# Hongje/OTVM

Hardware: AMD Instinct MI355X
Metric: frames_per_sec (higher is better)
Workload: dtype f16x3 (fp32 operands split into fp16 hi+lo, fp32 accumulate); 1 GPU; synthetic 1920x1080 clip, T=140 frames (untimed lead-in 0 + warmup 5 + timed: the last 135), memory every 5, max 5 slots, trimap propagation + alpha + memorize per frame, one sequence per GPU; weights=synthetic (otvm_amd.synth_weights seed 0), parallelism=sequence-per-gpu x1, batch=1

## Files before the change

### otvm_amd/csrc/gram.hip

```cpp
#include "common.h"
#include "f16x3_ops.h"
#include <stdlib.h>

namespace {

struct GramArgs {
    const float* x; int64_t P; int C, ld;
    const float* in_scale; const float* in_shift; float in_slope;
    float* gpart; float* spart;
    int nk, pch, nblk, nb;
    int64_t x_bs, g_bs, s_bs; int norm_bs;
    unsigned* diag;
};

constexpr int LDT = 40;

template <int BS, int PASSES>
__global__ __launch_bounds__(BS == 256 ? 512 : 256, BS == 256 ? 1 : 2) void gram_f16_kernel(const GramArgs pa) {
    GramArgs p = pa;
    {
        const int zb = blockIdx.y;
        p.x += zb * p.x_bs;
        p.gpart += zb * p.g_bs;
        p.spart += zb * p.s_bs;
        if (p.in_scale) { p.in_scale += zb * p.norm_bs; p.in_shift += zb * p.norm_bs; }
    }
    const int xcd = blockIdx.x & 7, slot = blockIdx.x >> 3;
    const int kc = xcd + 8 * (slot / p.nblk), blk = slot % p.nblk;
    if (kc >= p.nk) return;
    constexpr int NT = BS == 256 ? 512 : 256;
    constexpr int WM = BS == 256 ? 4 : 2, WN = 2;
    constexpr int TM = BS / (32 * WM), TN = BS / (32 * WN);
    constexpr int ROWS = 2 * BS;
    constexpr int STAGE = ROWS * LDT * (PASSES == 3 ? 2 : 1);
    __shared__ __attribute__((aligned(16))) _Float16 smem[2 * STAGE];
    const int tid = threadIdx.x, lane = tid & 63, wave = tid >> 6, wm = wave / WN, wn = wave % WN;
    int bi = 0, bj = 0;
    {
        int b = blk;
        while (b >= p.nb - bi) { b -= p.nb - bi; ++bi; }
        bj = bi + b;
    }
    const bool diag = bi == bj;
    const int boff = diag ? 0 : BS;
    const int64_t p0 = (int64_t)kc * p.pch;
    const int64_t p1 = p0 + p.pch < p.P ? p0 + p.pch : p.P;
    const int nchunks = (int)((p1 - p0 + 31) >> 5);

    constexpr int MAXIT = ((2 * BS / 4) * 8 + NT - 1) / NT;
    const int NQ = (diag ? BS : 2 * BS) / 4;
    const int pg = tid & 7;
    int row0[MAXIT], chan[MAXIT];
    bool live[MAXIT];
    f32x4 sc[MAXIT], sh[MAXIT], ssum[MAXIT];
#pragma unroll
    for (int k = 0; k < MAXIT; ++k) {
        const int cq = (tid >> 3) + (NT / 8) * k;
        live[k] = cq < NQ;
        row0[k] = cq * 4;
        chan[k] = live[k] ? (cq * 4 < BS ? bi * BS + cq * 4 : bj * BS + cq * 4 - BS) : 0;
        sc[k] = f32x4{1.f, 1.f, 1.f, 1.f};
        sh[k] = f32x4{0.f, 0.f, 0.f, 0.f};
        if (p.in_scale && live[k]) {
            sc[k] = *reinterpret_cast<const f32x4*>(p.in_scale + chan[k]);
            sh[k] = *reinterpret_cast<const f32x4*>(p.in_shift + chan[k]);
        }
        ssum[k] = f32x4{0.f, 0.f, 0.f, 0.f};
    }
    constexpr int PF = 2;
    f32x4 rg[PF][MAXIT][4];
    auto load_chunk = [&](int c, f32x4 (&r)[MAXIT][4]) __attribute__((always_inline)) {
#pragma unroll
        for (int k = 0; k < MAXIT; ++k)
#pragma unroll
            for (int i = 0; i < 4; ++i) {
                int64_t px = p0 + (int64_t)c * 32 + pg * 4 + i;
                px = px < p1 ? px : p1 - 1;
                r[k][i] = *reinterpret_cast<const f32x4*>(p.x + px * p.ld + chan[k]);
            }
    };
    bool sat = false;
    auto store_chunk = [&](int c, int buf, f32x4 (&r)[MAXIT][4]) __attribute__((always_inline)) {
        _Float16* Th = smem + buf * STAGE;
        _Float16* Tl = Th + ROWS * LDT;
#pragma unroll
        for (int k = 0; k < MAXIT; ++k) {
            if (!live[k]) continue;
            f32x4 v[4];
#pragma unroll
            for (int i = 0; i < 4; ++i) {
                const bool ok = p0 + (int64_t)c * 32 + pg * 4 + i < p1;
                f32x4 t = r[k][i] * sc[k] + sh[k];
                t.x = t.x > 0.f ? t.x : t.x * p.in_slope; t.y = t.y > 0.f ? t.y : t.y * p.in_slope;
                t.z = t.z > 0.f ? t.z : t.z * p.in_slope; t.w = t.w > 0.f ? t.w : t.w * p.in_slope;
                const f32x4 z = {0.f, 0.f, 0.f, 0.f};
                t = ok ? t : z;
                const f32x4 c4 = {__builtin_amdgcn_fmed3f(t.x, -65504.f, 65504.f), __builtin_amdgcn_fmed3f(t.y, -65504.f, 65504.f),
                                  __builtin_amdgcn_fmed3f(t.z, -65504.f, 65504.f), __builtin_amdgcn_fmed3f(t.w, -65504.f, 65504.f)};
                sat |= (c4.x != t.x) | (c4.y != t.y) | (c4.z != t.z) | (c4.w != t.w);
                v[i] = c4;
                ssum[k] += v[i];
            }
#pragma unroll
            for (int j = 0; j < 4; ++j) {
                const f16x4 hi = {(_Float16)v[0][j], (_Float16)v[1][j], (_Float16)v[2][j], (_Float16)v[3][j]};
                *reinterpret_cast<f16x4*>(&Th[(row0[k] + j) * LDT + pg * 4]) = hi;
                if (PASSES == 3) {
                    const f16x4 lo = {(_Float16)(v[0][j] - (float)hi.x), (_Float16)(v[1][j] - (float)hi.y),
                                      (_Float16)(v[2][j] - (float)hi.z), (_Float16)(v[3][j] - (float)hi.w)};
                    *reinterpret_cast<f16x4*>(&Tl[(row0[k] + j) * LDT + pg * 4]) = lo;
                }
            }
        }
    };
    f32x16 acc[TM][TN];
#pragma unroll
    for (int a = 0; a < TM; ++a)
#pragma unroll
        for (int b = 0; b < TN; ++b)
#pragma unroll
            for (int e = 0; e < 16; ++e) acc[a][b][e] = 0.f;
    auto compute = [&](int buf) __attribute__((always_inline)) {
        const _Float16* Th = smem + buf * STAGE;
        const _Float16* Tl = Th + ROWS * LDT;
        const int frow = lane & 31, fk = (lane >> 5) * 8;
#pragma unroll
        for (int ks = 0; ks < 2; ++ks) {
            f16x8 ah[TM], bh[TN], al[TM], bl[TN];
#pragma unroll
            for (int a = 0; a < TM; ++a) {
                const int o = ((wm * TM + a) * 32 + frow) * LDT + 16 * ks + fk;
                ah[a] = *reinterpret_cast<const f16x8*>(&Th[o]);
                if (PASSES == 3) al[a] = *reinterpret_cast<const f16x8*>(&Tl[o]);
            }
#pragma unroll
            for (int b = 0; b < TN; ++b) {
                const int o = (boff + (wn * TN + b) * 32 + frow) * LDT + 16 * ks + fk;
                bh[b] = *reinterpret_cast<const f16x8*>(&Th[o]);
                if (PASSES == 3) bl[b] = *reinterpret_cast<const f16x8*>(&Tl[o]);
            }
            if (PASSES == 3) {
#pragma unroll
                for (int a = 0; a < TM; ++a)
#pragma unroll
                    for (int b = 0; b < TN; ++b) acc[a][b] = __builtin_amdgcn_mfma_f32_32x32x16_f16(al[a], bh[b], acc[a][b], 0, 0, 0);
#pragma unroll
                for (int a = 0; a < TM; ++a)
#pragma unroll
                    for (int b = 0; b < TN; ++b) acc[a][b] = __builtin_amdgcn_mfma_f32_32x32x16_f16(ah[a], bl[b], acc[a][b], 0, 0, 0);
            }
#pragma unroll
            for (int a = 0; a < TM; ++a)
#pragma unroll
                for (int b = 0; b < TN; ++b) acc[a][b] = __builtin_amdgcn_mfma_f32_32x32x16_f16(ah[a], bh[b], acc[a][b], 0, 0, 0);
        }
    };

    if (nchunks > 0) {
        load_chunk(0, rg[0]);
        load_chunk(1, rg[1]);
        store_chunk(0, 0, rg[0]);
        load_chunk(2, rg[0]);
        __syncthreads();
        for (int c = 0; c < nchunks; c += PF) {
#pragma unroll
            for (int j = 0; j < PF; ++j) {
                if (c + j >= nchunks) break;
                compute((c + j) & 1);
                if (c + j + 1 < nchunks) store_chunk(c + j + 1, (c + j + 1) & 1, rg[(j + 1) % PF]);
                load_chunk(c + j + 3, rg[(j + 1) % PF]);
                __syncthreads();
            }
        }
    }
    if (sat && p.diag) atomicOr(p.diag + 1, 2u);
    float* gp = p.gpart + ((int64_t)kc * p.nblk + blk) * (BS * BS);
    const int col = lane & 31, rbase = (lane >> 5) * 4;
#pragma unroll
    for (int a = 0; a < TM; ++a)
#pragma unroll
        for (int b = 0; b < TN; ++b)
#pragma unroll
            for (int e = 0; e < 16; ++e) {
                const int m = (wm * TM + a) * 32 + (e & 3) + 8 * (e >> 2) + rbase, n = (wn * TN + b) * 32 + col;
                gp[m * BS + n] = acc[a][b][e];
            }
    if (diag) {
#pragma unroll
        for (int k = 0; k < MAXIT; ++k) {
            f32x4 s = ssum[k];
#pragma unroll
            for (int off = 1; off < 8; off <<= 1) {
                s.x += __shfl_xor(s.x, off); s.y += __shfl_xor(s.y, off); s.z += __shfl_xor(s.z, off); s.w += __shfl_xor(s.w, off);
            }
            if (live[k] && pg == 0) *reinterpret_cast<f32x4*>(p.spart + (int64_t)kc * p.C + chan[k]) = s;
        }
    }
}

struct PredArgs {
    const float* gpart; const float* spart; int nk, E, C;
    const float* Mp; const double* v;
    double* ws; unsigned* counter;
    int64_t P; int Cout;
    const float* wscale; const float* gamma; const float* beta; const float* res_shift;
    float* scale_eff; float* bias_eff; float* stat_out;
    int64_t g_bs, s_bs; int ws_bs, tab_bs, rs_bs;
    unsigned* diag;
};

constexpr int PRED_WG = 1024;
constexpr int PRED_KP = 4;
__global__ __launch_bounds__(256) void gn_predict_kernel(const PredArgs pa) {
    PredArgs p = pa;
    const int zb = blockIdx.y;
    p.gpart += zb * p.g_bs;
    p.spart += zb * p.s_bs;
    p.ws += (int64_t)zb * p.ws_bs;
    const int tid = threadIdx.x, lane = tid & 63, kp = tid >> 6;
    __shared__ double part[PRED_KP][64][4];
    __shared__ double red[4][64];
    __shared__ float t_mean[32], t_rstd[32];
    __shared__ unsigned t_last;
    const int nq = p.E >> 2;
    double a2[8] = {0.0, 0.0, 0.0, 0.0, 0.0, 0.0, 0.0, 0.0};
    for (int q0 = blockIdx.x * 64; q0 < nq; q0 += gridDim.x * 64) {
        const int q = q0 + lane;
        const float* gp = p.gpart + 4 * (int64_t)q;
        double s4[4] = {0.0, 0.0, 0.0, 0.0};
        for (int k0 = kp; k0 < p.nk; k0 += 8 * PRED_KP) {
            f32x4 u[8];
#pragma unroll
            for (int j = 0; j < 8; ++j) {
                const int kk = k0 + j * PRED_KP;
                u[j] = *reinterpret_cast<const f32x4*>(gp + (int64_t)(kk < p.nk ? kk : p.nk - 1) * p.E);
            }
#pragma unroll
            for (int j = 0; j < 8; ++j) {
                if (k0 + j * PRED_KP < p.nk) {
                    s4[0] += (double)u[j].x; s4[1] += (double)u[j].y; s4[2] += (double)u[j].z; s4[3] += (double)u[j].w;
                }
            }
        }
        __syncthreads();
#pragma unroll
        for (int j = 0; j < 4; ++j) part[kp][lane][j] = s4[j];
        __syncthreads();
        double g4[4];
#pragma unroll
        for (int j = 0; j < 4; ++j) g4[j] = (part[0][lane][j] + part[1][lane][j]) + (part[2][lane][j] + part[3][lane][j]);
        f32x4 m[8];
#pragma unroll
        for (int j = 0; j < 8; ++j) m[j] = *reinterpret_cast<const f32x4*>(p.Mp + (int64_t)(kp * 8 + j) * p.E + 4 * (int64_t)q);
#pragma unroll
        for (int j = 0; j < 8; ++j)
            a2[j] += (g4[0] * (double)m[j].x + g4[1] * (double)m[j].y) + (g4[2] * (double)m[j].z + g4[3] * (double)m[j].w);
    }
    double a1[8] = {0.0, 0.0, 0.0, 0.0, 0.0, 0.0, 0.0, 0.0};
    if ((int)blockIdx.x * 64 < p.C) {
        const int c = blockIdx.x * 64 + lane;
        double sv = 0.0;
        if (c < p.C)
            for (int k = kp; k < p.nk; k += PRED_KP) sv += (double)p.spart[(int64_t)k * p.C + c];
        __syncthreads();
        part[kp][lane][0] = sv;
        __syncthreads();
        const double st = (part[0][lane][0] + part[1][lane][0]) + (part[2][lane][0] + part[3][lane][0]);
        if (c < p.C) {
#pragma unroll
            for (int j = 0; j < 8; ++j) a1[j] = st * p.v[(int64_t)(kp * 8 + j) * p.C + c];
        }
    }
#pragma unroll
    for (int j = 0; j < 8; ++j) {
        double x = a2[j], y = a1[j];
#pragma unroll
        for (int off = 32; off > 0; off >>= 1) {
            x += __shfl_xor(x, off);
            y += __shfl_xor(y, off);
        }
        if (lane == 0) { red[0][2 * (kp * 8 + j)] = y; red[0][2 * (kp * 8 + j) + 1] = x; }
    }
    __syncthreads();
    if (tid < 64) __hip_atomic_store(p.ws + (int64_t)blockIdx.x * 64 + tid, red[0][tid], __ATOMIC_RELAXED, __HIP_MEMORY_SCOPE_AGENT);
    __builtin_amdgcn_fence(__ATOMIC_RELEASE, "workgroup");
    __builtin_amdgcn_s_waitcnt(0);
    __syncthreads();
    if (tid == 0) t_last = atomicAdd(p.counter + zb, 1u) == gridDim.x - 1 ? 1u : 0u;
    __syncthreads();
    if (!t_last) return;
    {
        const int vi = tid & 63, ph = tid >> 6, n = (int)gridDim.x;
        double t = 0.0;
        for (int w0 = ph; w0 < n; w0 += 32) {
            double u[8];
#pragma unroll
            for (int j = 0; j < 8; ++j) {
                const int w = w0 + 4 * j;
                u[j] = __hip_atomic_load(p.ws + (int64_t)(w < n ? w : n - 1) * 64 + vi, __ATOMIC_RELAXED, __HIP_MEMORY_SCOPE_AGENT);
            }
#pragma unroll
            for (int j = 0; j < 8; ++j)
                if (w0 + 4 * j < n) t += u[j];
        }
        red[ph][vi] = t;
    }
    __syncthreads();
    const int cg = p.Cout / 32;
    if (tid < 32) {
        const double cnt = (double)p.P * cg;
        const double sum = (red[0][2 * tid] + red[1][2 * tid]) + (red[2][2 * tid] + red[3][2 * tid]);
        const double sq = (red[0][2 * tid + 1] + red[1][2 * tid + 1]) + (red[2][2 * tid + 1] + red[3][2 * tid + 1]);
        const double mean = sum / cnt;
        double var = sq / cnt - mean * mean;
        if (var < 0.0) var = 0.0;
        t_mean[tid] = (float)mean;
        t_rstd[tid] = (float)(1.0 / sqrt(var + 1e-5));
        if (p.diag) {
            const double kappa = mean * mean / (var + 1e-12);
            const bool bad = !(sum == sum) || !(sq == sq) || !(fabs(sum) < 1e300) || !(fabs(sq) < 1e300);
            if (bad) atomicOr(p.diag + 1, 1u);
            else atomicMax(p.diag, __float_as_uint((float)(kappa < 3e38 ? kappa : 3e38)));
        }
        if (p.stat_out) { p.stat_out[zb * 64 + 2 * tid] = t_mean[tid]; p.stat_out[zb * 64 + 2 * tid + 1] = t_rstd[tid]; }
    }
    __syncthreads();
    float* se = p.scale_eff + (int64_t)zb * p.tab_bs;
    float* be = p.bias_eff + (int64_t)zb * p.tab_bs;
    const float* rs = p.res_shift ? p.res_shift + (int64_t)zb * p.rs_bs : nullptr;
    for (int c = tid; c < p.Cout; c += 256) {
        const int g = c / cg;
        const float a = t_rstd[g] * p.gamma[c];
        se[c] = p.wscale[c] * a;
        float b = p.beta[c] - t_mean[g] * a;
        if (rs) b += rs[c];
        be[c] = b;
    }
    if (tid == 0) __hip_atomic_store(p.counter + zb, 0u, __ATOMIC_RELAXED, __HIP_MEMORY_SCOPE_AGENT);
}

}

extern "C" int otvm_gram_block(int C) {
    static const int cap = otvm_probe_int("OTVM_GRAM_BS", 128);
    if (C % 256 == 0 && cap >= 256) return 256;
    return C % 128 == 0 && cap >= 128 ? 128 : 64;
}

extern "C" int64_t otvm_gram_entries(int C) {
    const int bs = otvm_gram_block(C), nb = C / bs;
    return (int64_t)(nb * (nb + 1) / 2) * bs * bs;
}

extern "C" int otvm_gram_chunks(int64_t P, int C, int* pch_out) {
    const int bs = otvm_gram_block(C), nb = C / bs, nblk = nb * (nb + 1) / 2;
    static const int wgs = otvm_probe_int("OTVM_GRAM_WGS", 0);
    int64_t nk = (wgs > 0 ? wgs : (bs == 256 ? 192 : 384)) / nblk;
    if (nk > 128) nk = 128;
    if (nk > P / 256) nk = P / 256;
    if (nk < (P + 1023) / 1024) nk = (P + 1023) / 1024;
    if (nk < 1) nk = 1;
    int64_t pch = (P + nk - 1) / nk;
    pch = (pch + 31) / 32 * 32;
    nk = (P + pch - 1) / pch;
    if (pch_out) *pch_out = (int)pch;
    return (int)nk;
}

extern "C" int64_t otvm_gn_predict_ws_bytes(void) { return (int64_t)PRED_WG * 64 * sizeof(double); }

extern "C" int otvm_gram_f16(const otvm_gram_params* q, void* stream) {
    OTVM_REQUIRE(q && q->x && q->gpart && q->spart, "otvm_gram_f16: null pointer");
    OTVM_REQUIRE(q->C % 64 == 0 && q->C >= 64 && q->ld % 4 == 0 && q->ld >= q->C && ((uintptr_t)q->x & 15) == 0,
                 "otvm_gram_f16: C must be a multiple of 64 in a 16-byte aligned view (C %d, ld %d)", q->C, q->ld);
    OTVM_REQUIRE(!q->in_scale == !q->in_shift, "otvm_gram_f16: in_scale and in_shift go together");
    OTVM_REQUIRE(q->passes == 1 || q->passes == 3, "otvm_gram_f16: passes must be 1 (fp16) or 3 (f16x3)");
    GramArgs a;
    a.x = q->x; a.P = q->P; a.C = q->C; a.ld = q->ld;
    a.in_scale = q->in_scale; a.in_shift = q->in_shift;
    a.in_slope = q->in_act == OTVM_ACT_RELU ? 0.f : (q->in_act == OTVM_ACT_LEAKY ? 0.01f : 1.f);
    a.gpart = q->gpart; a.spart = q->spart;
    const int bs = otvm_gram_block(q->C);
    a.nb = q->C / bs; a.nblk = a.nb * (a.nb + 1) / 2;
    int pch = 0;
    a.nk = otvm_gram_chunks(q->P, q->C, &pch);
    a.pch = pch;
    const int batch = q->batch > 1 ? q->batch : 1;
    a.x_bs = batch > 1 ? q->x_bs : 0; a.norm_bs = batch > 1 ? q->norm_bs : 0;
    a.g_bs = (int64_t)a.nk * otvm_gram_entries(q->C); a.s_bs = (int64_t)a.nk * q->C;
    a.diag = q->diag;
    const dim3 grid(a.nblk * ((a.nk + 7) / 8) * 8, batch);
    hipStream_t s = (hipStream_t)stream;
    const bool p3 = q->passes == 3;
    if (bs == 256) {
        if (p3) hipLaunchKernelGGL((gram_f16_kernel<256, 3>), grid, dim3(512), 0, s, a);
        else hipLaunchKernelGGL((gram_f16_kernel<256, 1>), grid, dim3(512), 0, s, a);
    } else if (bs == 128) {
        if (p3) hipLaunchKernelGGL((gram_f16_kernel<128, 3>), grid, dim3(256), 0, s, a);
        else hipLaunchKernelGGL((gram_f16_kernel<128, 1>), grid, dim3(256), 0, s, a);
    } else {
        if (p3) hipLaunchKernelGGL((gram_f16_kernel<64, 3>), grid, dim3(256), 0, s, a);
        else hipLaunchKernelGGL((gram_f16_kernel<64, 1>), grid, dim3(256), 0, s, a);
    }
    OTVM_CHECK_LAUNCH("otvm_gram_f16");
    return 0;
}

extern "C" int otvm_gn_predict(const otvm_gn_predict_params* q, void* stream) {
    OTVM_REQUIRE(q && q->gpart && q->spart && q->Mp && q->v && q->ws && q->counter && q->wscale && q->gamma && q->beta &&
                     q->scale_eff && q->bias_eff, "otvm_gn_predict: null pointer");
    OTVM_REQUIRE(q->Cout % 32 == 0 && q->C % 64 == 0, "otvm_gn_predict: Cout must be a multiple of 32 (got %d)", q->Cout);
    OTVM_REQUIRE(((uintptr_t)q->Mp & 15) == 0 && ((uintptr_t)q->gpart & 15) == 0, "otvm_gn_predict: Mp / gpart must be 16-byte aligned");
    PredArgs a;
    a.gpart = q->gpart; a.spart = q->spart; a.C = q->C;
    a.E = (int)otvm_gram_entries(q->C);
    a.nk = otvm_gram_chunks(q->P, q->C, nullptr);
    a.Mp = q->Mp; a.v = q->v; a.ws = (double*)q->ws; a.counter = q->counter;
    a.P = q->P; a.Cout = q->Cout;
    a.wscale = q->wscale; a.gamma = q->gamma; a.beta = q->beta; a.res_shift = q->res_shift;
    a.scale_eff = q->scale_eff; a.bias_eff = q->bias_eff; a.stat_out = q->stat_out;
    const int batch = q->batch > 1 ? q->batch : 1;
    a.g_bs = (int64_t)a.nk * a.E; a.s_bs = (int64_t)a.nk * q->C;
    a.ws_bs = PRED_WG * 64; a.tab_bs = batch > 1 ? q->tab_bs : 0; a.rs_bs = batch > 1 ? q->rs_bs : 0;
    a.diag = q->diag;
    int nwg = a.E / 256;
    if (nwg > 192) nwg = 192;
    if (nwg < otvm_ceil_div(a.C, 64)) nwg = otvm_ceil_div(a.C, 64);
    hipLaunchKernelGGL(gn_predict_kernel, dim3(nwg, batch), dim3(256), 0, (hipStream_t)stream, a);
    OTVM_CHECK_LAUNCH("otvm_gn_predict");
    return 0;
}
```

Measured before the change: 48.55 frames/s.

## Split GN-predict reduction over K chunks and retune gram prefetch and chunking

The gn_predict kernel now splits its reduction over gram chunks across more workgroups, spreading the per-channel sum work over several split groups and prefetching Mp, spart and v early. The final reduction gets wider phases, and affine parameters are preloaded before the last-block wait. The gram kernel gets a configurable prefetch depth per block size, 3 waves per SIMD for BS=128, and a halved block when BS equals C. The chunk-count heuristic now targets resident occupancy. Together these aim to raise parallelism and cut latency in the GroupNorm statistic prediction, at the cost of register pressure and more partial sums.

Result: no change. 48.86 frames/s, median of 6 (+0.6%).

```diff
diff --git a/otvm_amd/csrc/gram.hip b/otvm_amd/csrc/gram.hip
--- a/otvm_amd/csrc/gram.hip
+++ b/otvm_amd/csrc/gram.hip
@@ -13,10 +13,20 @@
     unsigned* diag;
 };
 
+#ifndef OTVM_GRAM_PF64
+#define OTVM_GRAM_PF64 2
+#endif
+#ifndef OTVM_GRAM_PF128
+#define OTVM_GRAM_PF128 1
+#endif
+#ifndef OTVM_GRAM_WG128
+#define OTVM_GRAM_WG128 3
+#endif
+constexpr int GRAM_PF(int bs) { return bs == 64 ? OTVM_GRAM_PF64 : (bs == 128 ? OTVM_GRAM_PF128 : 2); }
 constexpr int LDT = 40;
 
 template <int BS, int PASSES>
-__global__ __launch_bounds__(BS == 256 ? 512 : 256, BS == 256 ? 1 : 2) void gram_f16_kernel(const GramArgs pa) {
+__global__ __launch_bounds__(BS == 256 ? 512 : 256, BS == 256 ? 1 : (BS == 128 ? OTVM_GRAM_WG128 : 2)) void gram_f16_kernel(const GramArgs pa) {
     GramArgs p = pa;
     {
         const int zb = blockIdx.y;
@@ -67,7 +77,7 @@
         }
         ssum[k] = f32x4{0.f, 0.f, 0.f, 0.f};
     }
-    constexpr int PF = 2;
+    constexpr int PF = GRAM_PF(BS);
     f32x4 rg[PF][MAXIT][4];
     auto load_chunk = [&](int c, f32x4 (&r)[MAXIT][4]) __attribute__((always_inline)) {
 #pragma unroll
@@ -157,10 +167,10 @@
     };
 
     if (nchunks > 0) {
-        load_chunk(0, rg[0]);
-        load_chunk(1, rg[1]);
+#pragma unroll
+        for (int j = 0; j < PF; ++j) load_chunk(j, rg[j]);
         store_chunk(0, 0, rg[0]);
-        load_chunk(2, rg[0]);
+        load_chunk(PF, rg[0]);
         __syncthreads();
         for (int c = 0; c < nchunks; c += PF) {
 #pragma unroll
@@ -168,7 +178,7 @@
                 if (c + j >= nchunks) break;
                 compute((c + j) & 1);
                 if (c + j + 1 < nchunks) store_chunk(c + j + 1, (c + j + 1) & 1, rg[(j + 1) % PF]);
-                load_chunk(c + j + 3, rg[(j + 1) % PF]);
+                load_chunk(c + j + 1 + PF, rg[(j + 1) % PF]);
                 __syncthreads();
             }
         }
@@ -200,6 +210,8 @@
 
 struct PredArgs {
     const float* gpart; const float* spart; int nk, E, C;
+    int nqb, ksplit, kper;
+    int kss, kper_s;
     const float* Mp; const double* v;
     double* ws; unsigned* counter;
     int64_t P; int Cout;
@@ -210,7 +222,13 @@
 };
 
 constexpr int PRED_WG = 1024;
+constexpr int PRED_ITEMS = 768;
+constexpr int PRED_SPLIT_WG = 128;
+constexpr int PRED_KMIN = 32;
 constexpr int PRED_KP = 4;
+constexpr int PRED_TP = 8;
+constexpr int PRED_TB = 16;
+constexpr int PRED_TQ = 8;
 __global__ __launch_bounds__(256) void gn_predict_kernel(const PredArgs pa) {
     PredArgs p = pa;
     const int zb = blockIdx.y;
@@ -219,25 +237,49 @@
     p.ws += (int64_t)zb * p.ws_bs;
     const int tid = threadIdx.x, lane = tid & 63, kp = tid >> 6;
     __shared__ double part[PRED_KP][64][4];
-    __shared__ double red[4][64];
+    __shared__ double red[PRED_TP][64];
     __shared__ float t_mean[32], t_rstd[32];
     __shared__ unsigned t_last;
-    const int nq = p.E >> 2;
+    const int ncb = p.C >> 6;
+    const bool has_s = (int)blockIdx.x < ncb * p.kss;
+    const float* sp = p.spart;
+    int s_lo = 0, s_hi = 1;
+    float us[8] = {0.f, 0.f, 0.f, 0.f, 0.f, 0.f, 0.f, 0.f};
+    double vv[8] = {0.0, 0.0, 0.0, 0.0, 0.0, 0.0, 0.0, 0.0};
+    if (has_s) {
+        const int c = ((int)blockIdx.x % ncb) * 64 + lane;
+        const int k_lo = ((int)blockIdx.x / ncb) * p.kper_s;
+        s_lo = k_lo + kp;
+        s_hi = k_lo + p.kper_s < p.nk ? k_lo + p.kper_s : p.nk;
+        sp += c;
+#pragma unroll
+        for (int j = 0; j < 8; ++j) {
+            const int kk = s_lo + j * PRED_KP;
+            us[j] = sp[(int64_t)(kk < s_hi ? kk : s_hi - 1) * p.C];
+        }
+#pragma unroll
+        for (int j = 0; j < 8; ++j) vv[j] = p.v[(int64_t)(kp * 8 + j) * p.C + c];
+    }
     double a2[8] = {0.0, 0.0, 0.0, 0.0, 0.0, 0.0, 0.0, 0.0};
-    for (int q0 = blockIdx.x * 64; q0 < nq; q0 += gridDim.x * 64) {
-        const int q = q0 + lane;
+    const int items = p.nqb * p.ksplit;
+    for (int it = blockIdx.x; it < items; it += gridDim.x) {
+        const int q = (it % p.nqb) * 64 + lane;
+        const int k_lo = (it / p.nqb) * p.kper, k_hi = k_lo + p.kper < p.nk ? k_lo + p.kper : p.nk;
+        f32x4 m[8];
+#pragma unroll
+        for (int j = 0; j < 8; ++j) m[j] = *reinterpret_cast<const f32x4*>(p.Mp + (int64_t)(kp * 8 + j) * p.E + 4 * (int64_t)q);
         const float* gp = p.gpart + 4 * (int64_t)q;
         double s4[4] = {0.0, 0.0, 0.0, 0.0};
-        for (int k0 = kp; k0 < p.nk; k0 += 8 * PRED_KP) {
+        for (int k0 = k_lo + kp; k0 < k_hi; k0 += 8 * PRED_KP) {
             f32x4 u[8];
 #pragma unroll
             for (int j = 0; j < 8; ++j) {
                 const int kk = k0 + j * PRED_KP;
-                u[j] = *reinterpret_cast<const f32x4*>(gp + (int64_t)(kk < p.nk ? kk : p.nk - 1) * p.E);
+                u[j] = *reinterpret_cast<const f32x4*>(gp + (int64_t)(kk < k_hi ? kk : k_hi - 1) * p.E);
             }
 #pragma unroll
             for (int j = 0; j < 8; ++j) {
-                if (k0 + j * PRED_KP < p.nk) {
+                if (k0 + j * PRED_KP < k_hi) {
                     s4[0] += (double)u[j].x; s4[1] += (double)u[j].y; s4[2] += (double)u[j].z; s4[3] += (double)u[j].w;
                 }
             }
@@ -249,27 +291,33 @@
         double g4[4];
 #pragma unroll
         for (int j = 0; j < 4; ++j) g4[j] = (part[0][lane][j] + part[1][lane][j]) + (part[2][lane][j] + part[3][lane][j]);
-        f32x4 m[8];
-#pragma unroll
-        for (int j = 0; j < 8; ++j) m[j] = *reinterpret_cast<const f32x4*>(p.Mp + (int64_t)(kp * 8 + j) * p.E + 4 * (int64_t)q);
 #pragma unroll
         for (int j = 0; j < 8; ++j)
             a2[j] += (g4[0] * (double)m[j].x + g4[1] * (double)m[j].y) + (g4[2] * (double)m[j].z + g4[3] * (double)m[j].w);
     }
     double a1[8] = {0.0, 0.0, 0.0, 0.0, 0.0, 0.0, 0.0, 0.0};
-    if ((int)blockIdx.x * 64 < p.C) {
-        const int c = blockIdx.x * 64 + lane;
+    if (has_s) {
         double sv = 0.0;
-        if (c < p.C)
-            for (int k = kp; k < p.nk; k += PRED_KP) sv += (double)p.spart[(int64_t)k * p.C + c];
+#pragma unroll
+        for (int j = 0; j < 8; ++j)
+            if (s_lo + j * PRED_KP < s_hi) sv += (double)us[j];
+        for (int k0 = s_lo + 8 * PRED_KP; k0 < s_hi; k0 += 8 * PRED_KP) {
+            float u[8];
+#pragma unroll
+            for (int j = 0; j < 8; ++j) {
+                const int kk = k0 + j * PRED_KP;
+                u[j] = sp[(int64_t)(kk < s_hi ? kk : s_hi - 1) * p.C];
+            }
+#pragma unroll
+            for (int j = 0; j < 8; ++j)
+                if (k0 + j * PRED_KP < s_hi) sv += (double)u[j];
+        }
         __syncthreads();
         part[kp][lane][0] = sv;
         __syncthreads();
         const double st = (part[0][lane][0] + part[1][lane][0]) + (part[2][lane][0] + part[3][lane][0]);
-        if (c < p.C) {
-#pragma unroll
-            for (int j = 0; j < 8; ++j) a1[j] = st * p.v[(int64_t)(kp * 8 + j) * p.C + c];
-        }
+#pragma unroll
+        for (int j = 0; j < 8; ++j) a1[j] = st * vv[j];
     }
 #pragma unroll
     for (int j = 0; j < 8; ++j) {
@@ -289,28 +337,46 @@
     if (tid == 0) t_last = atomicAdd(p.counter + zb, 1u) == gridDim.x - 1 ? 1u : 0u;
     __syncthreads();
     if (!t_last) return;
+    const int cg = p.Cout / 32;
+    float* se = p.scale_eff + (int64_t)zb * p.tab_bs;
+    float* be = p.bias_eff + (int64_t)zb * p.tab_bs;
+    const float* rs = p.res_shift ? p.res_shift + (int64_t)zb * p.rs_bs : nullptr;
+    float tg[PRED_TQ], tb[PRED_TQ], tw[PRED_TQ], tr[PRED_TQ];
+#pragma unroll
+    for (int i = 0; i < PRED_TQ; ++i) {
+        const int c = tid + 256 * i < p.Cout ? tid + 256 * i : 0;
+        tg[i] = p.gamma[c]; tb[i] = p.beta[c]; tw[i] = p.wscale[c];
+        tr[i] = rs ? rs[c] : 0.f;
+    }
     {
-        const int vi = tid & 63, ph = tid >> 6, n = (int)gridDim.x;
-        double t = 0.0;
-        for (int w0 = ph; w0 < n; w0 += 32) {
-            double u[8];
-#pragma unroll
-            for (int j = 0; j < 8; ++j) {
-                const int w = w0 + 4 * j;
-                u[j] = __hip_atomic_load(p.ws + (int64_t)(w < n ? w : n - 1) * 64 + vi, __ATOMIC_RELAXED, __HIP_MEMORY_SCOPE_AGENT);
-            }
-#pragma unroll
-            for (int j = 0; j < 8; ++j)
-                if (w0 + 4 * j < n) t += u[j];
-        }
-        red[ph][vi] = t;
+        const int g = tid & 31, ph = tid >> 5, n = (int)gridDim.x;
+        const int n1 = ncb * p.kss < n ? ncb * p.kss : n;
+        auto column = [&](int vi, int cnt) __attribute__((always_inline)) {
+            double t = 0.0;
+            for (int w0 = ph; w0 < cnt; w0 += PRED_TB * PRED_TP) {
+                double u[PRED_TB];
+#pragma unroll
+                for (int j = 0; j < PRED_TB; ++j) {
+                    const int w = w0 + PRED_TP * j;
+                    u[j] = __hip_atomic_load(p.ws + (int64_t)(w < cnt ? w : cnt - 1) * 64 + vi, __ATOMIC_RELAXED, __HIP_MEMORY_SCOPE_AGENT);
+                }
+#pragma unroll
+                for (int j = 0; j < PRED_TB; ++j)
+                    if (w0 + PRED_TP * j < cnt) t += u[j];
+            }
+            return t;
+        };
+        __syncthreads();
+        red[ph][2 * g] = column(2 * g, n1);
+        red[ph][2 * g + 1] = column(2 * g + 1, n);
     }
     __syncthreads();
-    const int cg = p.Cout / 32;
     if (tid < 32) {
         const double cnt = (double)p.P * cg;
-        const double sum = (red[0][2 * tid] + red[1][2 * tid]) + (red[2][2 * tid] + red[3][2 * tid]);
-        const double sq = (red[0][2 * tid + 1] + red[1][2 * tid + 1]) + (red[2][2 * tid + 1] + red[3][2 * tid + 1]);
+        auto phases = [&](int vi) __attribute__((always_inline)) {
+            return ((red[0][vi] + red[1][vi]) + (red[2][vi] + red[3][vi])) + ((red[4][vi] + red[5][vi]) + (red[6][vi] + red[7][vi]));
+        };
+        const double sum = phases(2 * tid), sq = phases(2 * tid + 1);
         const double mean = sum / cnt;
         double var = sq / cnt - mean * mean;
         if (var < 0.0) var = 0.0;
@@ -325,10 +391,19 @@
         if (p.stat_out) { p.stat_out[zb * 64 + 2 * tid] = t_mean[tid]; p.stat_out[zb * 64 + 2 * tid + 1] = t_rstd[tid]; }
     }
     __syncthreads();
-    float* se = p.scale_eff + (int64_t)zb * p.tab_bs;
-    float* be = p.bias_eff + (int64_t)zb * p.tab_bs;
-    const float* rs = p.res_shift ? p.res_shift + (int64_t)zb * p.rs_bs : nullptr;
-    for (int c = tid; c < p.Cout; c += 256) {
+#pragma unroll
+    for (int i = 0; i < PRED_TQ; ++i) {
+        const int c = tid + 256 * i;
+        if (c < p.Cout) {
+            const int g = c / cg;
+            const float a = t_rstd[g] * tg[i];
+            se[c] = tw[i] * a;
+            float b = tb[i] - t_mean[g] * a;
+            if (rs) b += tr[i];
+            be[c] = b;
+        }
+    }
+    for (int c = tid + 256 * PRED_TQ; c < p.Cout; c += 256) {
         const int g = c / cg;
         const float a = t_rstd[g] * p.gamma[c];
         se[c] = p.wscale[c] * a;
@@ -343,8 +418,9 @@
 
 extern "C" int otvm_gram_block(int C) {
     static const int cap = otvm_probe_int("OTVM_GRAM_BS", 128);
-    if (C % 256 == 0 && cap >= 256) return 256;
-    return C % 128 == 0 && cap >= 128 ? 128 : 64;
+    int bs = C % 256 == 0 && cap >= 256 ? 256 : (C % 128 == 0 && cap >= 128 ? 128 : 64);
+    if (bs == C && bs > 64) bs >>= 1;
+    return bs;
 }
 
 extern "C" int64_t otvm_gram_entries(int C) {
@@ -355,14 +431,17 @@
 extern "C" int otvm_gram_chunks(int64_t P, int C, int* pch_out) {
     const int bs = otvm_gram_block(C), nb = C / bs, nblk = nb * (nb + 1) / 2;
     static const int wgs = otvm_probe_int("OTVM_GRAM_WGS", 0);
-    int64_t nk = (wgs > 0 ? wgs : (bs == 256 ? 192 : 384)) / nblk;
-    if (nk > 128) nk = 128;
-    if (nk > P / 256) nk = P / 256;
-    if (nk < (P + 1023) / 1024) nk = (P + 1023) / 1024;
+    const int64_t aim = ((wgs > 0 ? wgs : (bs == 256 ? 192 : 512)) + nblk - 1) / nblk;
+    const int64_t resident = 32 * (bs == 64 ? 4 : (bs == 128 ? OTVM_GRAM_WG128 : 1));
+    auto clamped = [](int64_t pch) { return pch < 128 ? (int64_t)128 : (pch > 1024 ? (int64_t)1024 : pch); };
+    int64_t pch = clamped(P / aim / 32 * 32);
+    int64_t nk = (P + pch - 1) / pch;
+    if (wgs <= 0 && (nk + 7) / 8 * nblk > resident && resident >= nblk) {
+        const int64_t fit = 8 * (resident / nblk);
+        pch = clamped(((P + fit - 1) / fit + 31) / 32 * 32);
+        nk = (P + pch - 1) / pch;
+    }
     if (nk < 1) nk = 1;
-    int64_t pch = (P + nk - 1) / nk;
-    pch = (pch + 31) / 32 * 32;
-    nk = (P + pch - 1) / pch;
     if (pch_out) *pch_out = (int)pch;
     return (int)nk;
 }
@@ -423,9 +502,21 @@
     a.g_bs = (int64_t)a.nk * a.E; a.s_bs = (int64_t)a.nk * q->C;
     a.ws_bs = PRED_WG * 64; a.tab_bs = batch > 1 ? q->tab_bs : 0; a.rs_bs = batch > 1 ? q->rs_bs : 0;
     a.diag = q->diag;
-    int nwg = a.E / 256;
-    if (nwg > 192) nwg = 192;
-    if (nwg < otvm_ceil_div(a.C, 64)) nwg = otvm_ceil_div(a.C, 64);
+    a.nqb = a.E / 256;
+    const int kmax = a.nk / PRED_KMIN > 1 ? a.nk / PRED_KMIN : 1;
+    int ksplit = (int)otvm_probe_int("OTVM_PRED_KSPLIT", 0);
+    if (ksplit <= 0) ksplit = PRED_SPLIT_WG / a.nqb < kmax ? PRED_SPLIT_WG / a.nqb : kmax;
+    if (ksplit > a.nk) ksplit = a.nk;
+    if (ksplit < 1) ksplit = 1;
+    a.kper = otvm_ceil_div(a.nk, ksplit);
+    a.ksplit = otvm_ceil_div(a.nk, a.kper);
+    const int ncb = a.C / 64;
+    int nwg = a.nqb * a.ksplit < PRED_ITEMS ? a.nqb * a.ksplit : PRED_ITEMS;
+    if (nwg < ncb) nwg = ncb;
+    const int kss = nwg / ncb < kmax ? nwg / ncb : kmax;
+    a.kper_s = otvm_ceil_div(a.nk, kss);
+    a.kss = otvm_ceil_div(a.nk, a.kper_s);
+    OTVM_REQUIRE(nwg <= PRED_WG && ncb * a.kss <= nwg, "otvm_gn_predict: %d workgroups for %d rows of workspace", nwg, PRED_WG);
     hipLaunchKernelGGL(gn_predict_kernel, dim3(nwg, batch), dim3(256), 0, (hipStream_t)stream, a);
     OTVM_CHECK_LAUNCH("otvm_gn_predict");
     return 0;
```
